# Genesis-Embodied-AI/ThinShellLab

Hardware: AMD Instinct MI355X
Metric: element-steps/s (fwd+adjoint), 100k-tri cloth; 1/2/4/8-GPU scaling (higher is better)
Workload: dtype f64

## Files before the change

### thinshelllab_amd/csrc/direct_host.hpp

```cpp
#pragma once
#include <array>
#include <chrono>

#include "k_direct.hpp"
#include "tsl_ctx.hpp"

#include <cerrno>
#include <fcntl.h>
#include <sys/file.h>
#include <sys/stat.h>
#include <unistd.h>
static void ds_flow_token_acquire(DirectSolver& d) {
  char bus[64] = "dev";
  if (hipDeviceGetPCIBusId(bus, sizeof(bus), d.device) != hipSuccess) { (void)hipGetLastError(); snprintf(bus, sizeof(bus), "dev%d", d.device); }
  for (char* q = bus; *q; q++) if (*q == ':' || *q == '/') *q = '_';
  d.flow_token = -1; d.flow_token_asked = d.n_factor;
  for (const char* dir : {"/dev/shm", "/tmp"}) {
    const std::string path = std::string(dir) + "/tsl_flow_" + bus;
    int fd = open(path.c_str(), O_RDWR | O_CLOEXEC);
    if (fd < 0 && errno == ENOENT) {
      fd = open(path.c_str(), O_CREAT | O_RDWR | O_CLOEXEC, 0666);
      if (fd < 0 && (errno == ENOENT || errno == ENOTDIR)) continue;
      if (fd < 0 && errno == EEXIST) fd = open(path.c_str(), O_RDWR | O_CLOEXEC);
    } else if (fd < 0 && errno == ENOTDIR) continue;
// ... 285 lines not shown
  if (d.cache_cap > 0) {
    const uint64_t key = ds_cons_key(cset);
    HIP_OK(hipStreamSynchronize(s));
    for (auto& sl : d.cache)
      if (sl->used && sl->key == key && sl->h_cset == cset) {
        ds_swap_slot(d, *sl);
        sl->used = d.plan_valid; sl->key = ds_cons_key(sl->h_cset); sl->stamp = ++d.cache_clock;
        d.plan_valid = true;
        d.n_plan_hits++; d.plan_gen++;
        if (c->group) TSL_TRY(group_ensure_arenas(c));
        if (c->verbose >= 2) fprintf(stderr, "[tsl] direct plan: cached plan reused (nc %d, %d supernodes)\n", c->nc, d.plan.sym.n_sn);
        return same_set_new_order();
      }
    if (d.plan_valid) {
      DsPlanSlot* dst = nullptr;
      for (auto& sl : d.cache) if (!sl->used) { dst = sl.get(); break; }
      if (!dst && (int)d.cache.size() < d.cache_cap) {
        d.cache.emplace_back(new DsPlanSlot());
        dst = d.cache.back().get();
        dst->plan.sym.copy_partition(d.plan.sym); dst->plan.threads = d.plan.threads; dst->plan.n_cu = d.plan.n_cu; dst->plan.split_small = d.plan.split_small; dst->plan.split_rem = d.plan.split_rem;
      }
      if (!dst) { for (auto& sl : d.cache) if (!dst || sl->stamp < dst->stamp) dst = sl.get(); }
      ds_swap_slot(d, *dst);
      dst->used = true; dst->key = ds_cons_key(dst->h_cset); dst->stamp = ++d.cache_clock;
      d.plan_valid = false;
      ds_cache_trim(d);
    }
  }
  const auto t0 = std::chrono::steady_clock::now();
  const int rc = d.plan.build(c->h_rows, d.row_ptr, cons.data(), c->nc);
  const auto t_build = std::chrono::steady_clock::now();
  if (rc) return tsl_fail("direct solver: inconsistent elimination tree (code %d)", rc);
  DirectPlan& P = d.plan;
  std::vector<int> vtxp(P.vtx.size());
  for (size_t i = 0; i < vtxp.size(); i++) vtxp[i] = c->h_rowpos[P.vtx[i]];
  HIP_OK(hipStreamSynchronize(s));
  const size_t nbk = P.blk_q.size();
  ds_pin_reset(d, 16 * nbk + 2 * sizeof(DsFrontDesc) * P.fr.size() + sizeof(DsChildRec) * P.ch_rec.size() +
                      4 * (P.level_sn.size() + P.pmap.size() + vtxp.size() + P.wl_front.size() + P.wl_row.size()) + 20 * (P.cgr_ent.size() + P.cgr_ptr.size()) + 64 * 256);
  TSL_TRY(ds_upload_grow(d.fr, P.fr, s, &d)); TSL_TRY(ds_upload_grow(d.level_sn, P.level_sn, s, &d)); TSL_TRY(ds_upload_grow(d.pmap, P.pmap, s, &d)); TSL_TRY(ds_upload_grow(d.ch_rec, P.ch_rec, s, &d));
  TSL_TRY(ds_upload_grow(d.vtx, vtxp, s, &d));
  {
    std::vector<int> src_v, ld_v;
    std::vector<long long> dst_v;
    int* src_l = (int*)ds_pin_take(d, 4 * nbk); int* ld_l = (int*)ds_pin_take(d, 4 * nbk); long long* dst_l = (long long*)ds_pin_take(d, 8 * nbk);
    if (!src_l || !ld_l || !dst_l) { src_v.resize(nbk); ld_v.resize(nbk); dst_v.resize(nbk); src_l = src_v.data(); ld_l = ld_v.data(); dst_l = dst_v.data(); }
    ds_parallel_for((int)((nbk + 4095) / 4096), P.n_threads(), 1, [&](int, int ch) {
      for (size_t i = (size_t)ch * 4096; i < std::min(nbk, (size_t)(ch + 1) * 4096); i++) { const int q = P.blk_q[i]; src_l[i] = d.h_c2s[q]; dst_l[i] = P.blk_dst[q]; ld_l[i] = P.blk_ld[q]; }
    });
    if (d.blk_dst.n < nbk) { if (d.blk_dst.alloc(nbk + nbk / 4 + 16)) return -1; }
    if (d.blk_ld.n < nbk) { if (d.blk_ld.alloc(nbk + nbk / 4 + 16)) return -1; }
    if (d.blk_q.n < nbk) { if (d.blk_q.alloc(nbk + nbk / 4 + 16)) return -1; }
    if (nbk > 0) {
      HIP_OK(hipMemcpyAsync(d.blk_dst.p, dst_l, 8 * nbk, hipMemcpyHostToDevice, s));
      HIP_OK(hipMemcpyAsync(d.blk_ld.p, ld_l, 4 * nbk, hipMemcpyHostToDevice, s));
      HIP_OK(hipMemcpyAsync(d.blk_q.p, src_l, 4 * nbk, hipMemcpyHostToDevice, s));
      if (!src_v.empty()) HIP_OK(hipStreamSynchronize(s));
    }
  }
  TSL_TRY(ds_upload_con(d, s));
  std::vector<DsFrontDesc> frl(P.level_sn.size());
  for (size_t i = 0; i < frl.size(); i++) frl[i] = P.fr[P.level_sn[i]];
  TSL_TRY(ds_upload_grow(d.frl, frl, s, &d));
  TSL_TRY(ds_upload_grow(d.wl_front, P.wl_front, s, &d)); TSL_TRY(ds_upload_grow(d.wl_row, P.wl_row, s, &d));
  if (c->group) TSL_TRY(group_ensure_arenas(c));
  else {
    if (d.prezero_pending && d.arena.n < (size_t)P.arena) { HIP_OK(hipEventSynchronize(d.ev_zero)); d.prezero_pending = false; }
    if (d.arena.n < (size_t)P.arena) { if (d.arena.alloc((size_t)P.arena + (size_t)P.arena / 8)) return tsl_fail("direct solver: out of device memory (%.2f GB of front panels)", P.arena * 8e-9); }
    if (d.sarena.n < (size_t)P.sarena) { if (d.sarena.alloc((size_t)P.sarena + (size_t)P.sarena / 8 + 16)) return tsl_fail("direct solver: out of device memory (%.2f GB of Schur complements)", P.sarena * 8e-9); }
    if (d.garena.n < (size_t)P.garena) { if (d.garena.alloc((size_t)P.garena + (size_t)P.garena / 8 + 16)) return tsl_fail("direct solver: out of device memory (G arena)"); }
    if (d.w.n < (size_t)P.ylen) { if (d.w.alloc((size_t)P.ylen + (size_t)P.ylen / 4 + 16)) return -1; }
  }
  if (d.scr.n < (size_t)P.scratch) { if (d.scr.alloc((size_t)P.scratch + (size_t)P.scratch / 8)) return -1; }
  HIP_OK(hipStreamSynchronize(s));
  d.h_cons.swap(cons); d.h_cset.swap(cset);
  d.plan_valid = true;
  d.numeric_valid = false;
  d.have_factor = false;
  d.n_plans++; d.plan_gen++;
  d.t_plan += std::chrono::duration<double>(std::chrono::steady_clock::now() - t0).count();
  if (c->verbose >= 2)
    fprintf(stderr, "[tsl] direct plan: %d supernodes, %d levels, %zu batches, %.2f + %.2f GB of panels + Schur complements, %.1f GFLOP per factorisation, nc %d; host %.2f ms (tree + maps %.2f)\n", P.sym.n_sn, P.n_levels, P.batches.size(), P.arena * 8e-9, P.sarena * 8e-9,
            P.flops * 1e-9, c->nc, 1e3 * std::chrono::duration<double>(std::chrono::steady_clock::now() - t0).count(), 1e3 * std::chrono::duration<double>(t_build - t0).count());
  if (c->verbose >= 2) fprintf(stderr, "[tsl]   plan phases (ms): tree %.2f, descriptors + parent maps %.2f, levels %.2f, static block map %.2f, contact map %.2f\n", P.phase_ms[0], P.phase_ms[1], P.phase_ms[2], P.phase_ms[3], P.phase_ms[4]);
  if (c->verbose >= 3)
    for (const DsBatch& b : P.batches) {
      fprintf(stderr, "[tsl]   level %2d: %5d fronts, pivots <= %4d, boundary <= %4d%s; fronts by padded pivot count:", b.level, b.count, b.max_pp, b.max_bp, ds_use_small(d, b) ? " (LDS kernel)" : "");
      for (int q = 0, run = 0; q < b.count; q++) {
        run++;
        if (q + 1 == b.count || P.fr[P.level_sn[b.first + q + 1]].pp != P.fr[P.level_sn[b.first + q]].pp) { fprintf(stderr, " %d x %d", run, P.fr[P.level_sn[b.first + q]].pp); run = 0; }
      }
      fprintf(stderr, "\n");
    }
  return 0;
}

static int direct_prezero(tsl_ctx* c) {
  DirectSolver& d = c->ds;
  if (!d.prezero || !d.plan_valid || d.arena.n == 0 || d.prezero_pending) return 0;
  if (d.zstream == nullptr) {
    HIP_OK(hipStreamCreateWithFlags(&d.zstream, hipStreamNonBlocking));
    HIP_OK(hipEventCreateWithFlags(&d.ev_zfork, hipEventDisableTiming));
    HIP_OK(hipEventCreateWithFlags(&d.ev_zero, hipEventDisableTiming));
  }
  HIP_OK(hipEventRecord(d.ev_zfork, c->stream));
  HIP_OK(hipStreamWaitEvent(d.zstream, d.ev_zfork, 0));
  d.prezero_n = (size_t)d.plan.arena_leaf;
  if (d.plan.leaf_ranges.empty()) HIP_OK(hipMemsetAsync(d.arena.p, 0, d.prezero_n * sizeof(double), d.zstream));
  else for (const auto& r : d.plan.leaf_ranges) HIP_OK(hipMemsetAsync(d.arena.p + r.first, 0, (size_t)r.second * sizeof(double), d.zstream));
  HIP_OK(hipEventRecord(d.ev_zero, d.zstream));
  d.prezero_pending = true;
  d.numeric_valid = false; d.have_factor = false;
  return 0;
}

static void ds_launch_gemv(hipStream_t s, const DsDev& D, DirectSolver& d, int o, int n, int mode, const double* vin, double* vout, int wide_from = -1) {
  if (n <= 0) return;
  if (wide_from >= 0) {
    const int n0 = wide_from - o, n1 = o + n - wide_from;
    if (n0 > 0) hipLaunchKernelGGL(k_ds_gemv, dim3(n0), dim3(256), 0, s, D, d.wl_front.p, d.wl_row.p, o, mode, vin, vout);
    if (n1 > 0) hipLaunchKernelGGL(k_ds_gemv_wide, dim3(4 * n1), dim3(256), 0, s, D, d.wl_front.p, d.wl_row.p, wide_from, mode, vin, vout);
    return;
  }
  if (d.gemv_wide_below > 0 && n < d.gemv_wide_below) hipLaunchKernelGGL(k_ds_gemv_wide, dim3(4 * n), dim3(256), 0, s, D, d.wl_front.p, d.wl_row.p, o, mode, vin, vout);
  else hipLaunchKernelGGL(k_ds_gemv, dim3(n), dim3(256), 0, s, D, d.wl_front.p, d.wl_row.p, o, mode, vin, vout);
}
static void ds_sweep_up_level(hipStream_t s, const DsDev& D, DirectSolver& d, int l, const double* r, double* z) {
  const DirectPlan& P = d.plan;
  const int o0 = P.wl_own_ptr[l], b0 = P.wl_bnd_ptr[l], o1 = P.wl_own_ptr[l + 1];
  ds_launch_gemv(s, D, d, o0, b0 - o0, 0, r, z, P.wl_own_wide.empty() ? -1 : P.wl_own_wide[l]);
  ds_launch_gemv(s, D, d, b0, o1 - b0, 1, (const double*)z, nullptr, P.wl_bnd_wide.empty() ? -1 : P.wl_bnd_wide[l]);
}
static int direct_factor(tsl_ctx* c, int stop_sn = -1, const char* dump_path = nullptr, const double* eager_r = nullptr, double* eager_z = nullptr) {
  DirectSolver& d = c->ds;
  hipStream_t s = c->stream;
  TSL_TRY(direct_plan(c));
  if (d.numeric_valid) return 0;
  d.eager_n = 0;
  const DirectPlan& P = d.plan;
  const DsDev D = ds_dev(c);
  if (d.prezero_pending) {
    HIP_OK(hipStreamWaitEvent(s, d.ev_zero, 0));
    d.prezero_pending = false;
    if (P.leaf_ranges.empty() && d.prezero_n < (size_t)P.arena_leaf) HIP_OK(hipMemsetAsync(d.arena.p + d.prezero_n, 0, ((size_t)P.arena_leaf - d.prezero_n) * sizeof(double), s));
  } else if (P.leaf_ranges.empty()) HIP_OK(hipMemsetAsync(d.arena.p, 0, (size_t)P.arena_leaf * sizeof(double), s));
  else for (const auto& r : P.leaf_ranges) HIP_OK(hipMemsetAsync(d.arena.p + r.first, 0, (size_t)r.second * sizeof(double), s));
  HIP_OK(hipMemsetAsync(d.bad.p, 0, 8 * sizeof(int), s));
  bool swept_at_root = false;
  int flow_wgs_sent = 0;
  auto invert_batch = [&](const DsBatch& b, hipStream_t bs, bool& flow_free) {
    const int lv0 = b.first, nf = b.count;
    const int tp = b.max_pp / DS_T;
    bool flowed = false;
    {
      const std::vector<DsBatch> pieces = ds_flow_pieces(d, P, b, flow_free, bs);
      std::vector<DsFlowArgs> fas(pieces.size());
      bool ready = !pieces.empty();
      for (size_t i = 0; ready && i < pieces.size(); i++) ready = ds_flow_prepare(d, P, pieces[i], true, fas[i], bs);
      if (ready) {
        for (size_t i = 0; i < pieces.size(); i++) { ds_flow_launch(bs, D, pieces[i].first, fas[i], d); d.n_flow++; flow_wgs_sent += fas[i].tile0[fas[i].nf]; }
        flowed = true; flow_free = false;
      }
    }
    if (flowed) {}
    else if (ds_use_small(d, b)) hipLaunchKernelGGL(k_ds_inv_small, dim3(nf), dim3(256), ds_small_lds(b.max_pp), bs, D, lv0, b.max_pp + 1);
    else {
      hipLaunchKernelGGL(k_ds_pivot0, dim3(nf), dim3(256), 0, bs, D, lv0);
      for (int k = 0; k < tp; k++) { const int na = P.act_n[b.act_off + k]; hipLaunchKernelGGL(k_ds_gj_step, dim3(na + na * tp * tp), dim3(256), 0, bs, D, lv0, k, tp, na); }
      hipLaunchKernelGGL(k_ds_gj_finish, dim3(tp, nf), dim3(256), 0, bs, D, lv0);
    }
  };
  auto run_batch = [&](const DsBatch& b, hipStream_t bs, bool& flow_free) {
    invert_batch(b, bs, flow_free);
    if (b.max_bp > 0) {
      ds_launch_gemm(bs, D, b, 0, d.xcd_map, d.g32_below);
      ds_launch_gemm(bs, D, b, 1, d.xcd_map);
    }
  };
  auto side_streams = [&]() -> int {
    if (d.fstream[0] == nullptr)
      for (int k = 0; k < DS_NSIDE; k++) { HIP_OK(hipStreamCreateWithFlags(&d.fstream[k], hipStreamNonBlocking)); HIP_OK(hipEventCreateWithFlags(&d.ev_fjoin[k], hipEventDisableTiming)); }
    if (d.ev_ffork == nullptr) HIP_OK(hipEventCreateWithFlags(&d.ev_ffork, hipEventDisableTiming));
    for (int k = 0; k < 5; k++) if (d.ev_la[k] == nullptr) HIP_OK(hipEventCreateWithFlags(&d.ev_la[k], hipEventDisableTiming));
    if (d.lastream == nullptr) {
      int lo = 0, hi = 0;
      HIP_OK(hipDeviceGetStreamPriorityRange(&lo, &hi));
      HIP_OK(hipStreamCreateWithPriority(&d.lastream, hipStreamNonBlocking, lo));
    }
    return 0;
  };
  const bool la_on = (d.lookahead & 1) && stop_sn < 0 && !P.blk_lmid.empty() && P.la_from < P.n_levels && ds_flow_token_held(d);
  if (la_on) TSL_TRY(side_streams());
  hipStream_t ls = d.lastream;
  enum { LA_W = 0, LA_GA = 1, LA_A = 2, LA_REST = 3, LA_DRAIN = 4 };
  for (size_t bi = 0; bi < P.batches.size();) {
    size_t be = bi;
    while (be < P.batches.size() && P.batches[be].level == P.batches[bi].level) be++;
    bool stop_here = false;
    if (stop_sn >= 0) for (int q = P.batches[bi].first; q < P.batches[be - 1].first + P.batches[be - 1].count; q++) stop_here |= P.level_sn[q] == stop_sn;
    const int lvl = P.batches[bi].level;
    const bool la_level = la_on && lvl >= P.la_from;
    const bool la_in = la_level && lvl > P.la_from;
    if (la_in) {
      ds_launch_level_start(c, s, D, lvl, 1, &P.batches[bi]);
      HIP_OK(hipStreamWaitEvent(ls, d.ev_la[LA_A], 0));
      ds_launch_level_start(c, ls, D, lvl, 2, &P.batches[bi]);
      HIP_OK(hipEventRecord(d.ev_la[LA_REST], ls));
    } else
    ds_launch_level_start(c, s, D, lvl);
    if (la_level) {
      const DsBatch& b = P.batches[bi];
      bool flow_free = true;
      if (la_in && ds_flow_wgs(P, b) > P.n_cu) {
        HIP_OK(hipEventRecord(d.ev_la[LA_DRAIN], ls));
        HIP_OK(hipStreamWaitEvent(s, d.ev_la[LA_DRAIN], 0));
      }
      invert_batch(b, s, flow_free);
      if (la_in && eager_r != nullptr && (d.lookahead & 2) && lvl >= P.n_levels - 3) {
        const int top = P.n_levels - 1;
        const int c0 = std::min((d.lookahead >> 2) & 7, top - 2);
        const int c1r = (d.lookahead >> 5) & 15, c1 = c1r == 0 ? top - 1 : std::min(std::max(c1r, c0), top - 1);
// ... 249 lines not shown
```

### thinshelllab_amd/csrc/direct_sym.hpp

```cpp
#pragma once
#include <algorithm>
#include <cstdint>
#include <cstdio>
#include <vector>

struct DsGrid { int v_offset, N, M; };
struct DsBlock { int v_offset, n_verts; };

struct DirectSym {
  int NV = 0;
  std::vector<int> c_order;
  std::vector<int> c_ptr;
  std::vector<int> c_lo;
  std::vector<int> c_grid;
  std::vector<int> c_pos;
  std::vector<int> c_sn;
  std::vector<DsBlock> blocks;
  std::vector<int> body_of;
  std::vector<std::vector<std::vector<int>>> b_sn;
  std::vector<int> loose;
  std::vector<int> order, epos, sn_of, sn_ptr;
  int n_sn = 0;
  int merge_sep = 16;
  bool merge_k = true;
  std::vector<std::vector<int>> bnd;
  std::vector<int> parent, level;
  int n_levels = 0;

  void copy_partition(const DirectSym& o) {
    NV = o.NV; c_order = o.c_order; c_ptr = o.c_ptr; c_lo = o.c_lo; c_grid = o.c_grid; c_pos = o.c_pos; c_sn = o.c_sn;
    blocks = o.blocks; body_of = o.body_of; b_sn = o.b_sn; loose = o.loose; merge_sep = o.merge_sep; merge_k = o.merge_k;
  }

  int own(int s) const { return sn_ptr[s + 1] - sn_ptr[s]; }

  int local(int s, int v) const {
    if (sn_of[v] == s) return epos[v] - sn_ptr[s];
    const auto& b = bnd[s];
    const int e = epos[v];
    int lo = 0, hi = (int)b.size();
    while (lo < hi) { const int m = (lo + hi) >> 1; if (epos[b[m]] < e) lo = m + 1; else hi = m; }
    if (lo < (int)b.size() && b[lo] == v) return own(s) + lo;
    return -1;
  }

  void build_partition(int nv, const std::vector<std::vector<int>>& adj, const std::vector<DsGrid>& grids, const std::vector<DsBlock>& blocks_in, int leaf_verts) {
    NV = nv;
    blocks = blocks_in;
    c_order.clear(); c_ptr.assign(1, 0); c_lo.clear(); c_grid.clear();
    c_pos.assign(nv, -1); c_sn.assign(nv, -1); body_of.assign(nv, -1); loose.clear();
    for (size_t b = 0; b < blocks.size(); b++)
      for (int v = blocks[b].v_offset; v < blocks[b].v_offset + blocks[b].n_verts; v++) body_of[v] = (int)b;
    b_sn.assign(blocks.size(), {});
    {
      std::vector<int> lab(nv, -1);
      for (size_t b = 0; b < blocks.size(); b++) {
        std::vector<int> region(blocks[b].n_verts);
        for (int k = 0; k < blocks[b].n_verts; k++) region[k] = blocks[b].v_offset + k;
        dissect_graph(adj, region, std::max(leaf_verts, 40), lab, b_sn[b]);
      }
    }
    std::vector<int> side(nv, 0);
    for (size_t gi = 0; gi < grids.size(); gi++) {
      const DsGrid& g = grids[gi];
      std::vector<int> region((size_t)(g.N + 1) * (g.M + 1));
      for (size_t k = 0; k < region.size(); k++) region[k] = g.v_offset + (int)k;
      dissect(g, (int)gi, adj, region, leaf_verts, side);
    }
    for (size_t q = 0; q < c_order.size(); q++) c_pos[c_order[q]] = (int)q;
    for (size_t s = 0; s + 1 < c_ptr.size(); s++)
      for (int q = c_ptr[s]; q < c_ptr[s + 1]; q++) c_sn[c_order[q]] = (int)s;
    for (int v = 0; v < nv; v++) if (c_pos[v] < 0 && body_of[v] < 0) loose.push_back(v);
  }

  void dissect_graph(const std::vector<std::vector<int>>& adj, std::vector<int>& region, int leaf, std::vector<int>& lab, std::vector<std::vector<int>>& out) {
    if (region.empty()) return;
    if ((int)region.size() <= leaf) { std::sort(region.begin(), region.end()); out.push_back(region); return; }
    std::vector<int> q;
    auto bfs = [&](int start) {
      for (int v : region) lab[v] = 0;
      q.clear(); q.push_back(start); lab[start] = 1;
      for (size_t h = 0; h < q.size(); h++)
        for (int u : adj[q[h]]) if (lab[u] == 0) { lab[u] = lab[q[h]] + 1; q.push_back(u); }
    };
    bfs(region[0]);
    if (q.size() < region.size()) {
      std::vector<int> comp(q), rest;
      for (int v : region) if (lab[v] == 0) rest.push_back(v);
      for (int v : region) lab[v] = -1;
      dissect_graph(adj, comp, leaf, lab, out);
      dissect_graph(adj, rest, leaf, lab, out);
      return;
    }
    bfs(q.back());
    const int nl = lab[q.back()];
    if (nl < 3) { for (int v : region) lab[v] = -1; std::sort(region.begin(), region.end()); out.push_back(region); return; }
    std::vector<int> cnt(nl + 2, 0);
    for (int v : region) cnt[lab[v]]++;
    int m = 2, acc = cnt[1];
    while (m < nl - 1 && 2 * (acc + cnt[m]) < (int)region.size()) { acc += cnt[m]; m++; }
    std::vector<int> A, B, S;
    for (int v : region) { if (lab[v] < m) A.push_back(v); else if (lab[v] > m) B.push_back(v); else S.push_back(v); }
    for (int v : region) lab[v] = -1;
    std::vector<int>().swap(region);
    dissect_graph(adj, A, leaf, lab, out);
    dissect_graph(adj, B, leaf, lab, out);
    std::sort(S.begin(), S.end());
    out.push_back(S);
  }

  void close_static(int lo, int grid) {
    if ((int)c_order.size() > c_ptr.back()) { c_ptr.push_back((int)c_order.size()); c_lo.push_back(lo); c_grid.push_back(grid); }
  }

  void dissect(const DsGrid& g, int gi, const std::vector<std::vector<int>>& adj, std::vector<int>& region, int leaf_verts, std::vector<int>& side, std::vector<int>* up = nullptr) {
    if (region.empty()) return;
    const int lo = (int)c_order.size();
    const int W = g.M + 1;
    int i0 = 1 << 30, i1 = -1, j0 = 1 << 30, j1 = -1;
    for (int v : region) { const int i = (v - g.v_offset) / W, j = (v - g.v_offset) % W; i0 = std::min(i0, i); i1 = std::max(i1, i); j0 = std::min(j0, j); j1 = std::max(j1, j); }
    const int ni = i1 - i0 + 1, nj = j1 - j0 + 1;
    if ((int)region.size() <= leaf_verts || (ni <= 3 && nj <= 3)) {
      std::sort(region.begin(), region.end());
      for (int v : region) c_order.push_back(v);
      close_static(lo, gi);
      return;
    }
    const bool along_i = ni >= nj;
    const int m = along_i ? (i0 + i1) / 2 : (j0 + j1) / 2;
    auto coord = [&](int v) { const int k = v - g.v_offset; return along_i ? k / W : k % W; };
    auto other = [&](int v) { const int k = v - g.v_offset; return along_i ? k % W : k / W; };
    std::vector<int> L, R, S;
    for (int v : region) { const int cv = coord(v); side[v] = cv < m ? 1 : cv > m + 1 ? 2 : 3; }
    std::vector<int> sep;
    for (int v : region) if (side[v] == 3) sep.push_back(v);
    std::stable_sort(sep.begin(), sep.end(), [&](int a, int b) { return coord(a) > coord(b); });
    for (int v : sep) {
      bool hasL = false, hasR = false;
      for (int u : adj[v]) { if (side[u] == 1) hasL = true; else if (side[u] == 2) hasR = true; }
      if (!hasL) side[v] = 2; else if (!hasR) side[v] = 1;
    }
    for (int v : region) { if (side[v] == 1) L.push_back(v); else if (side[v] == 2) R.push_back(v); else S.push_back(v); }
    for (int v : region) side[v] = 0;
    std::vector<int>().swap(region);
    std::vector<int> handed;
    dissect(g, gi, adj, L, leaf_verts, side, &handed);
    dissect(g, gi, adj, R, leaf_verts, side, &handed);
    std::sort(S.begin(), S.end(), [&](int a, int b) { return other(a) != other(b) ? other(a) < other(b) : coord(a) < coord(b); });
    if (up != nullptr && handed.empty() && (int)S.size() <= merge_sep) { up->insert(up->end(), S.begin(), S.end()); return; }
    for (int v : handed) c_order.push_back(v);
    for (int v : S) c_order.push_back(v);
    close_static(lo, gi);
  }

  void build_tree(const std::vector<std::vector<int>>& adj, const int* extra, int n_extra, int clique) {
    std::vector<std::vector<int>> xadj;
    std::vector<int> xidx(NV, -1);
    for (int e = 0; e < n_extra; e++)
      for (int a = 0; a < clique; a++) {
        const int va = extra[e * clique + a];
        if (xidx[va] < 0) { xidx[va] = (int)xadj.size(); xadj.emplace_back(); }
        for (int b = 0; b < clique; b++) if (b != a) xadj[xidx[va]].push_back(extra[e * clique + b]);
      }
    const int n_static = (int)c_ptr.size() - 1, END = n_static;
    const int nb = (int)blocks.size();
    std::vector<int> ins(nb, -1);
    std::vector<std::vector<int>> K(nb);
    for (int b = 0; b < nb; b++) {
      int pmin = 1 << 30, pmax = -1, grid = -1;
      bool to_end = false;
      for (int v = blocks[b].v_offset; v < blocks[b].v_offset + blocks[b].n_verts; v++) {
        if (xidx[v] < 0) continue;
        K[b].push_back(v);
        for (int u : xadj[xidx[v]]) {
          if (body_of[u] == b) continue;
          if (c_pos[u] < 0) { to_end = true; continue; }
          const int gu = c_grid[c_sn[u]];
          if (grid >= 0 && gu != grid) to_end = true;
          grid = gu;
          pmin = std::min(pmin, c_pos[u]); pmax = std::max(pmax, c_pos[u]);
        }
      }
      if (K[b].empty()) continue;
      if (to_end || pmax < 0) { ins[b] = END; continue; }
      int s = c_sn[c_order[pmax]];
      while (s < n_static && !(c_lo[s] <= pmin && c_ptr[s + 1] > pmax && c_grid[s] == grid)) s++;
      ins[b] = s;
    }
    order.clear(); sn_ptr.assign(1, 0);
    auto close_sn = [&]() { if ((int)order.size() > sn_ptr.back()) sn_ptr.push_back((int)order.size()); };
    for (int b = 0; b < nb; b++)
      for (const auto& sn : b_sn[b]) { for (int v : sn) if (xidx[v] < 0) order.push_back(v); close_sn(); }
    for (int v : loose) { order.push_back(v); close_sn(); }
    std::vector<std::vector<int>> at(n_static + 1);
    for (int b = 0; b < nb; b++) if (ins[b] >= 0) at[ins[b]].push_back(b);
    for (int s = 0; s <= n_static; s++) {
      for (int b : at[s]) for (int v : K[b]) order.push_back(v);
      if (!merge_k || s == n_static) close_sn();
      if (s < n_static) { for (int q = c_ptr[s]; q < c_ptr[s + 1]; q++) order.push_back(c_order[q]); close_sn(); }
    }
    n_sn = (int)sn_ptr.size() - 1;
    epos.assign(NV, 0); sn_of.assign(NV, 0);
    for (int p = 0; p < NV; p++) epos[order[p]] = p;
    for (int s = 0; s < n_sn; s++)
      for (int p = sn_ptr[s]; p < sn_ptr[s + 1]; p++) sn_of[order[p]] = s;
    bnd.assign(n_sn, {});
    parent.assign(n_sn, -1);
    level.assign(n_sn, 0);
    std::vector<std::vector<int>> children(n_sn);
    std::vector<int> mark(NV, -1);
    for (int s = 0; s < n_sn; s++) {
      std::vector<int>& b = bnd[s];
      auto visit = [&](int u) { if (sn_of[u] > s && mark[u] != s) { mark[u] = s; b.push_back(u); } };
      for (int p = sn_ptr[s]; p < sn_ptr[s + 1]; p++) {
        const int v = order[p];
        for (int u : adj[v]) visit(u);
        if (xidx[v] >= 0) for (int u : xadj[xidx[v]]) visit(u);
      }
      for (int c : children[s]) for (int u : bnd[c]) visit(u);
      std::sort(b.begin(), b.end(), [&](int x, int y) { return epos[x] < epos[y]; });
      if (!b.empty()) { parent[s] = sn_of[b[0]]; children[parent[s]].push_back(s); }
    }
    n_levels = 0;
    for (int s = 0; s < n_sn; s++) {
      int lv = 0;
      for (int c : children[s]) lv = std::max(lv, level[c] + 1);
      level[s] = lv;
      n_levels = std::max(n_levels, lv + 1);
    }
  }

  void stats(double* flops, double* front_doubles, int* max_front, int* max_p) const {
    double fl = 0, mem = 0;
    int mf = 0, mp = 0;
    for (int s = 0; s < n_sn; s++) {
      const double p = 3.0 * own(s), b = 3.0 * bnd[s].size();
      fl += 2.0 * p * p * p + 2.0 * p * p * b + 2.0 * p * b * b;
      mem += (p + b) * (p + b);
      mf = std::max(mf, (int)(p + b)); mp = std::max(mp, (int)p);
    }
    *flops = fl; *front_doubles = mem; *max_front = mf; *max_p = mp;
  }
};
```

### thinshelllab_amd/csrc/tsl_hip.hip

```cpp
#include <stdarg.h>
#include <cctype>
#include <chrono>
#include <mutex>

#include <array>
#include <map>

#include "k_cloth.hpp"
#include "k_contact.hpp"
#include "k_fem.hpp"
#include "k_mg.hpp"
#include "k_param.hpp"
#include "k_solver.hpp"
#include "tsl_ctx.hpp"

thread_local std::string g_tsl_err;
int tsl_fail(const char* fmt, ...) {
  char buf[1024];
  va_list ap;
  va_start(ap, fmt);
  vsnprintf(buf, sizeof(buf), fmt, ap);
  va_end(ap);
  g_tsl_err = buf;
  return -1;
// ... 1229 lines not shown
  if (c->nc > 0) std::swap(c->c_H.p, c->c_H_pc.p);
  const int rc = assemble(c, c->st_pos, c->st_prev, c->st_vel, c->st_ref, 2, nullptr);
  c->mg_omega_valid = false; c->mg_cinv_valid = false;
  c->bd_valid = false;
  int rc2 = 0;
  if (!rc) {
    if (body_active(c) && !c->bd_valid) rc2 = body_build_inverse(c);
    if (!rc2) rc2 = mg_setup_operators(c);
  }
  std::swap(c->vals.p, c->vals_pc.p);
  if (c->nc > 0) std::swap(c->c_H.p, c->c_H_pc.p);
  (void)s;
  if (rc || rc2) return -1;
  c->pc_separate = true;
  return 0;
}

static int ds_flow_lost(tsl_ctx* c, bool suspect, int note[8]) {
  const DirectSolver& d = c->ds;
  const bool forced = d.dbg == 21 || d.dbg == 22;
  if (!(suspect || forced) || !d.flow || d.n_flow <= 0) return 0;
  int ab = 0;
  HIP_OK(hipStreamSynchronize(c->stream));
  HIP_OK(hipMemcpy(&ab, d.bad.p + DS_FLOW_ABORT, sizeof(int), hipMemcpyDeviceToHost));
  if (!ab && !forced) return 0;
  for (int k = 0; k < 8; k++) note[k] = 0;
  (void)hipMemcpy(note, d.bad.p + DS_BAD_NOTE, 8 * sizeof(int), hipMemcpyDeviceToHost);
  return 1;
}

static int solve_perm(tsl_ctx* c, tsl_solve_stats* st, const tsl_solve_stats* first) {
  hipStream_t s = c->stream;
  const int NV = c->NV;
  const size_t n3 = 3 * (size_t)NV;
  const int gb = nblk(NV, 256);
  st->iters = 0; st->restarts = 0; st->flag = 0; st->rel_residual = 0; st->method = 0; st->attained = 0; st->backward_error = 0;
  c->last_xmax_valid = false;
  if (direct_enabled(c) && !c->ds_suspended) {
    DirectSolver& d = c->ds;
    if (!first && d.enable < 0 && !d.hard && c->n_tet == 0 && c->nc == 0) {
      c->ds_suspended = true; c->ds_probe = true;
      const int maxit_keep = c->cg_maxit;
      c->cg_maxit = std::min(c->cg_maxit, d.probe_cap);
      tsl_solve_stats s2;
      const int rc = solve_perm(c, &s2);
      c->cg_maxit = maxit_keep;
      c->ds_suspended = false; c->ds_probe = false;
      if (rc) return rc;
      if (s2.flag == 0) { *st = s2; return 0; }
      d.hard = true; d.hard_steps = 0;
      st->iters = s2.iters;
    }
    tsl_solve_stats sd = first ? *first : *st;
    auto direct_try = [&]() -> int {
      if (!d.numeric_valid) {
        TSL_TRY(direct_plan(c));
        TSL_TRY(direct_factor(c, -1, nullptr, c->v_b.p, c->v_x.p));
      }
      int rc_g = direct_refine(c, &sd, first != nullptr);
      if (rc_g == 0 && sd.flag != 1) { const int it0 = sd.iters; sd = *st; c->last_xmax_valid = false; rc_g = gmres(c, &sd, true); sd.iters += it0; }
      if (rc_g) return -1;
      int note[8];
      const int lost = ds_flow_lost(c, sd.flag != 1, note);
      if (lost < 0) return -1;
      if (lost) {
        const bool blame_la = (d.lookahead & 1) != 0 && d.n_flow_abort == 0 && d.dbg != 21;
        fprintf(stderr, "[tsl] k_ds_gj_flow: a workgroup waited in vain for a flag (launch not resident as a whole?): %s disabled for this context, refactorising "
                "(workgroup %d of %d gave up; %d of the %d workgroups of the factorisation's dataflow launches had started; flag value %d, epoch %d)\n",
                blame_la ? "\"direct_lookahead\"" : "\"direct_flow\"", note[2], note[1], note[0], d.flow_wgs_last, note[3], note[4]);
        const int flow_keep = d.flow;
        d.flow = 0; d.n_flow_abort++;
        if (blame_la) d.lookahead = 0;
        d.numeric_valid = false; d.have_factor = false;
        if (d.prezero_pending) { HIP_OK(hipStreamWaitEvent(c->stream, d.ev_zero, 0)); d.prezero_pending = false; }
        TSL_TRY(direct_factor(c));
        if (blame_la) d.flow = flow_keep;
        sd = *st; c->last_xmax_valid = false;
        TSL_TRY(direct_refine(c, &sd));
        if (sd.flag != 1) { const int it0 = sd.iters; sd = *st; c->last_xmax_valid = false; TSL_TRY(gmres(c, &sd, true)); sd.iters += it0; }
      }
      return 0;
    };
    if (direct_try() != 0) {
      if (d.enable == 1) return -1;
      (void)hipGetLastError();
      d.numeric_valid = false; d.have_factor = false; d.plan_valid = false;
      fprintf(stderr, "[tsl] direct solver set-up failed (%s): this solve runs on the iterative hierarchy%s\n", tsl_last_error(),
              ++d.n_setup_fail >= 3 ? "; direct path disabled for this context" : "");
      if (d.n_setup_fail >= 3) d.enable = 0;
      c->ds_suspended = true;
      const int rc = solve_perm(c, st);
      c->ds_suspended = false;
      if (rc == 0 && st->flag == 0) st->flag = 1;
      return rc;
    }
    if (sd.flag == 1) { *st = sd; st->flag = 0; st->method = 4; return 0; }
    if (c->verbose) {
      int nb[4] = {0, 0, 0, 0};
      (void)hipMemcpy(nb, d.bad.p, sizeof(nb), hipMemcpyDeviceToHost);
      fprintf(stderr, "[tsl] direct factorisation + GMRES did not converge (rel_residual %.2e, backward error %.2e after %d iterations, perturbed pivots %d / %d / %d in fronts of <= 128 / <= 512 / more pivots, nc %d): iterative fallback\n",
              sd.rel_residual, sd.backward_error, sd.iters, nb[1], nb[2], nb[3], c->nc);
      if (c->verbose > 1) {
        std::vector<int> lg(DS_BAD_NOTE);
        (void)hipMemcpy(lg.data(), d.bad.p, lg.size() * sizeof(int), hipMemcpyDeviceToHost);
        const int nl = std::min(lg[4], DS_BADLOG);
        static int n_dump = 0;
        if (const char* dir = getenv("TSL_DUMP_DIR")) if (nl > 0 && n_dump < 3) {
          char path[512];
          snprintf(path, sizeof(path), "%s/front_%d.bin", dir, n_dump++);
          d.numeric_valid = false;
          TSL_TRY(direct_factor(c, lg[8] >> 6, path));
        }
        for (int i = 0; i < nl; i++) {
          const int* L = &lg[8 + 4 * i];
          const int sn = L[0] >> 6, kt = L[0] & 63;
          const DsFrontDesc& f = d.plan.fr[sn];
          float am; memcpy(&am, L + 3, 4);
          const unsigned mask = (unsigned)L[1];
          const int first = __builtin_ctz(mask | 0x80000000u), row = kt * DS_T + first;
          const int vtx = row < f.p ? d.plan.vtx[f.vtx_off + row / 3] : -1;
          fprintf(stderr, "[tsl]   perturbed pivots: front %d (level %d, p %d, b %d, own verts %d) tile %d rows mask %08x, first row %d (vertex %d dof %d%s), tile max %.3e\n",
                  sn, d.plan.sym.level[sn], f.p, f.b, f.nv_own, kt, mask, row, vtx, row % 3, vtx >= 0 && d.plan.sym.body_of[vtx] >= 0 ? ", body" : "", am);
        }
      }
    }
    if (sd.rel_residual <= 1e-3) { *st = sd; st->flag = 3; st->method = 4; return 0; }
    c->ds_suspended = true;
    tsl_solve_stats s2;
    const int maxit_keep = c->cg_maxit;
    c->cg_maxit = std::min(c->cg_maxit, d.fallback_cap);
    HIP_OK(hipMemcpyAsync(c->v_t4.p, c->v_x.p, 3 * (size_t)c->NV * sizeof(double), hipMemcpyDeviceToDevice, c->stream));
    const int rc = solve_perm(c, &s2);
    c->cg_maxit = maxit_keep;
    c->ds_suspended = false;
    const bool sd_ok = std::isfinite(sd.rel_residual), s2_ok = rc == 0 && std::isfinite(s2.rel_residual);
    if (rc == 0 && s2.flag == 3 && !sd_ok && !s2_ok) return tsl_fail("linear solve: factorisation and iterative fallback both ended with a non-finite residual");
    if (rc == 0 && s2.flag == 3 && sd_ok && (!s2_ok || !(s2.rel_residual < sd.rel_residual))) {
      HIP_OK(hipMemcpyAsync(c->v_x.p, c->v_t4.p, 3 * (size_t)c->NV * sizeof(double), hipMemcpyDeviceToDevice, c->stream));
      *st = sd; st->iters = sd.iters + s2.iters; st->flag = 3; st->method = 4;
      return 0;
    }
    st->iters = sd.iters + s2.iters; st->restarts = s2.restarts + 1; st->rel_residual = s2.rel_residual; st->method = s2.method; st->attained = s2.attained;
    st->flag = s2.flag == 0 ? 1 : s2.flag;
    return rc;
  }
  TSL_TRY(block_jacobi_ensure(c));
  const bool warm = false;
  if (!warm) HIP_OK(hipMemsetAsync(c->v_x.p, 0, n3 * sizeof(double), s));
  HIP_OK(hipMemsetAsync(c->scal.p, 0, sizeof(SolverScalars), s));
  hipLaunchKernelGGL(k_dot, dim3(DOT_BLOCKS), dim3(256), 0, s, n3, c->v_b.p, c->v_b.p, &SC(c)->bb, DOT_SCRATCH(c));
  TSL_TRY(read_scal(c));
  const double bb = HSC(c)->bb;
  if (!(bb > 0)) return 0;
  const double tol2 = c->cg_tol * c->cg_tol * bb;
  bool need_fallback = false, indefinite = false;
  int total_it = 0;
  const int ncb = c->nc > 0 ? nblk(c->nc, 64) : 0;
  if (body_active(c) && !c->bd_valid) TSL_TRY(body_build_inverse(c));
  const bool bd = body_active(c) && c->bd_valid;
  const int n_rz = gb + (bd ? c->bd_wg : 0);
  double rr_prev_outer = 1e300;
  for (int outer = 0; outer < 20; outer++) {
    PcgScal hs;
    memset(&hs, 0, sizeof(hs));
    hs.bb = bb; hs.thresh2 = 0.25 * tol2; hs.n_part1 = c->n_slices; hs.n_part2 = n_rz;
    HIP_OK(hipMemcpyAsync(c->scal.p, &hs, sizeof(PcgScal), hipMemcpyHostToDevice, s));
// ... 1498 lines not shown
```

Baseline: 525,600.

## Reuse constraint-free elimination tree boundaries when rebuilding the direct solver plan

Caches the elimination tree and supernode boundary sets computed without contact constraints, and on each replan only recomputes boundaries for static supernodes touched by contact cliques and their ancestors. Clean supernodes copy their cached boundary lists, which is meant to cut host-side symbolic planning time per step. Scratch workspaces are kept across calls to avoid reallocations. It also adds a state check for when the cached tree applies, and resets eager_n earlier. The cost is added complexity and a correctness risk if the dirty propagation misses a case.

Result: no change. 522,000 (-0.7%).

```diff
diff --git a/thinshelllab_amd/csrc/direct_host.hpp b/thinshelllab_amd/csrc/direct_host.hpp
--- a/thinshelllab_amd/csrc/direct_host.hpp
+++ b/thinshelllab_amd/csrc/direct_host.hpp
@@ -391,7 +391,8 @@
   if (c->verbose >= 2)
     fprintf(stderr, "[tsl] direct plan: %d supernodes, %d levels, %zu batches, %.2f + %.2f GB of panels + Schur complements, %.1f GFLOP per factorisation, nc %d; host %.2f ms (tree + maps %.2f)\n", P.sym.n_sn, P.n_levels, P.batches.size(), P.arena * 8e-9, P.sarena * 8e-9,
             P.flops * 1e-9, c->nc, 1e3 * std::chrono::duration<double>(std::chrono::steady_clock::now() - t0).count(), 1e3 * std::chrono::duration<double>(t_build - t0).count());
-  if (c->verbose >= 2) fprintf(stderr, "[tsl]   plan phases (ms): tree %.2f, descriptors + parent maps %.2f, levels %.2f, static block map %.2f, contact map %.2f\n", P.phase_ms[0], P.phase_ms[1], P.phase_ms[2], P.phase_ms[3], P.phase_ms[4]);
+  if (c->verbose >= 1) fprintf(stderr, "[tsl]   plan phases (ms): tree %.2f (%d of %d boundaries kept from the constraint-free tree), descriptors + parent maps %.2f, levels %.2f, static block map %.2f, contact map %.2f, uploads %.2f\n",
+                               P.phase_ms[0], P.sym.n_reused, P.sym.n_sn, P.phase_ms[1], P.phase_ms[2], P.phase_ms[3], P.phase_ms[4], 1e3 * std::chrono::duration<double>(std::chrono::steady_clock::now() - t_build).count());
   if (c->verbose >= 3)
     for (const DsBatch& b : P.batches) {
       fprintf(stderr, "[tsl]   level %2d: %5d fronts, pivots <= %4d, boundary <= %4d%s; fronts by padded pivot count:", b.level, b.count, b.max_pp, b.max_bp, ds_use_small(d, b) ? " (LDS kernel)" : "");
@@ -443,9 +444,9 @@
 static int direct_factor(tsl_ctx* c, int stop_sn = -1, const char* dump_path = nullptr, const double* eager_r = nullptr, double* eager_z = nullptr) {
   DirectSolver& d = c->ds;
   hipStream_t s = c->stream;
+  d.eager_n = 0;
   TSL_TRY(direct_plan(c));
   if (d.numeric_valid) return 0;
-  d.eager_n = 0;
   const DirectPlan& P = d.plan;
   const DsDev D = ds_dev(c);
   if (d.prezero_pending) {
diff --git a/thinshelllab_amd/csrc/direct_sym.hpp b/thinshelllab_amd/csrc/direct_sym.hpp
--- a/thinshelllab_amd/csrc/direct_sym.hpp
+++ b/thinshelllab_amd/csrc/direct_sym.hpp
@@ -26,10 +26,18 @@
   std::vector<std::vector<int>> bnd;
   std::vector<int> parent, level;
   int n_levels = 0;
+  bool reuse = true;
+  int st_state = 0;
+  std::vector<int> st_parent;
+  std::vector<int> st_bptr, st_bnd;
+  int n_reused = 0;
+  std::vector<std::vector<int>> w_xadj, w_K, w_at, w_children;
+  std::vector<int> w_xidx, w_touched, w_ins, w_mark, w_dirty, w_dyn;
 
   void copy_partition(const DirectSym& o) {
     NV = o.NV; c_order = o.c_order; c_ptr = o.c_ptr; c_lo = o.c_lo; c_grid = o.c_grid; c_pos = o.c_pos; c_sn = o.c_sn;
     blocks = o.blocks; body_of = o.body_of; b_sn = o.b_sn; loose = o.loose; merge_sep = o.merge_sep; merge_k = o.merge_k;
+    reuse = o.reuse; st_state = o.st_state; st_parent = o.st_parent; st_bptr = o.st_bptr; st_bnd = o.st_bnd;
   }
 
   int own(int s) const { return sn_ptr[s + 1] - sn_ptr[s]; }
@@ -47,6 +55,7 @@
   void build_partition(int nv, const std::vector<std::vector<int>>& adj, const std::vector<DsGrid>& grids, const std::vector<DsBlock>& blocks_in, int leaf_verts) {
     NV = nv;
     blocks = blocks_in;
+    st_state = 0; st_parent.clear(); st_bptr.clear(); st_bnd.clear();
     c_order.clear(); c_ptr.assign(1, 0); c_lo.clear(); c_grid.clear();
     c_pos.assign(nv, -1); c_sn.assign(nv, -1); body_of.assign(nv, -1); loose.clear();
     for (size_t b = 0; b < blocks.size(); b++)
@@ -153,7 +162,7 @@
     close_static(lo, gi);
   }
 
-  void build_tree(const std::vector<std::vector<int>>& adj, const int* extra, int n_extra, int clique) {
+  void build_tree_scratch(const std::vector<std::vector<int>>& adj, const int* extra, int n_extra, int clique) {
     std::vector<std::vector<int>> xadj;
     std::vector<int> xidx(NV, -1);
     for (int e = 0; e < n_extra; e++)
@@ -230,6 +239,134 @@
     }
   }
 
+  void build_static_tree(const std::vector<std::vector<int>>& adj) {
+    const int n_static = (int)c_ptr.size() - 1;
+    st_state = -1;
+    if (!loose.empty() || n_static == 0) return;
+    for (int v = 0; v < NV; v++)
+      for (int u : adj[v]) if ((c_pos[v] >= 0) != (c_pos[u] >= 0) || body_of[v] != body_of[u]) return;
+    build_tree_scratch(adj, nullptr, 0, 4);
+    const int base = n_sn - n_static;
+    if (base < 0) return;
+    for (int s = 0; s < n_static; s++) if (sn_ptr[base + s + 1] - sn_ptr[base + s] != c_ptr[s + 1] - c_ptr[s] || order[sn_ptr[base + s]] != c_order[c_ptr[s]]) return;
+    st_parent.assign(n_static, -1); st_bptr.assign(n_static + 1, 0); st_bnd.clear();
+    for (int s = 0; s < n_static; s++) {
+      if (parent[base + s] >= 0) { if (parent[base + s] < base) return; st_parent[s] = parent[base + s] - base; }
+      for (int u : bnd[base + s]) { if (c_pos[u] < 0) return; st_bnd.push_back(u); }
+      st_bptr[s + 1] = (int)st_bnd.size();
+    }
+    st_state = 1;
+  }
+
+  void build_tree(const std::vector<std::vector<int>>& adj, const int* extra, int n_extra, int clique) {
+    n_reused = 0;
+    if (!reuse) { build_tree_scratch(adj, extra, n_extra, clique); return; }
+    if (st_state == 0) build_static_tree(adj);
+    if (st_state < 0) { build_tree_scratch(adj, extra, n_extra, clique); return; }
+    std::vector<std::vector<int>>& xadj = w_xadj;
+    std::vector<int>& xidx = w_xidx;
+    if ((int)xidx.size() != NV) { xidx.assign(NV, -1); w_touched.clear(); }
+    for (int v : w_touched) xidx[v] = -1;
+    w_touched.clear();
+    int nx = 0;
+    for (int e = 0; e < n_extra; e++)
+      for (int a = 0; a < clique; a++) {
+        const int va = extra[e * clique + a];
+        if (xidx[va] < 0) { xidx[va] = nx++; w_touched.push_back(va); if ((int)xadj.size() < nx) xadj.emplace_back(); xadj[nx - 1].clear(); }
+        for (int b = 0; b < clique; b++) if (b != a) xadj[xidx[va]].push_back(extra[e * clique + b]);
+      }
+    const int n_static = (int)c_ptr.size() - 1, END = n_static;
+    const int nb = (int)blocks.size();
+    std::vector<int>& ins = w_ins;
+    ins.assign(nb, -1);
+    std::vector<std::vector<int>>& K = w_K;
+    K.resize(nb);
+    for (int b = 0; b < nb; b++) {
+      K[b].clear();
+      int pmin = 1 << 30, pmax = -1, grid = -1;
+      bool to_end = false;
+      for (int v = blocks[b].v_offset; v < blocks[b].v_offset + blocks[b].n_verts; v++) {
+        if (xidx[v] < 0) continue;
+        K[b].push_back(v);
+        for (int u : xadj[xidx[v]]) {
+          if (body_of[u] == b) continue;
+          if (c_pos[u] < 0) { to_end = true; continue; }
+          const int gu = c_grid[c_sn[u]];
+          if (grid >= 0 && gu != grid) to_end = true;
+          grid = gu;
+          pmin = std::min(pmin, c_pos[u]); pmax = std::max(pmax, c_pos[u]);
+        }
+      }
+      if (K[b].empty()) continue;
+      if (to_end || pmax < 0) { ins[b] = END; continue; }
+      int s = c_sn[c_order[pmax]];
+      while (s < n_static && !(c_lo[s] <= pmin && c_ptr[s + 1] > pmax && c_grid[s] == grid)) s++;
+      ins[b] = s;
+    }
+    order.clear(); sn_ptr.assign(1, 0);
+    auto close_sn = [&]() { if ((int)order.size() > sn_ptr.back()) sn_ptr.push_back((int)order.size()); };
+    for (int b = 0; b < nb; b++)
+      for (const auto& sn : b_sn[b]) { for (int v : sn) if (xidx[v] < 0) order.push_back(v); close_sn(); }
+    for (int v : loose) { order.push_back(v); close_sn(); }
+    std::vector<std::vector<int>>& at = w_at;
+    at.resize(n_static + 1);
+    for (auto& a : at) a.clear();
+    for (int b = 0; b < nb; b++) if (ins[b] >= 0) at[ins[b]].push_back(b);
+    std::vector<int>& dyn = w_dyn;
+    dyn.clear();
+    for (int s = 0; s <= n_static; s++) {
+      for (int b : at[s]) for (int v : K[b]) order.push_back(v);
+      if (!merge_k || s == n_static) close_sn();
+      if (s < n_static) { for (int q = c_ptr[s]; q < c_ptr[s + 1]; q++) order.push_back(c_order[q]); close_sn(); dyn.resize(sn_ptr.size() - 1, -1); dyn.back() = s; }
+    }
+    n_sn = (int)sn_ptr.size() - 1;
+    dyn.resize(n_sn, -1);
+    epos.resize(NV); sn_of.resize(NV);
+    for (int p = 0; p < NV; p++) epos[order[p]] = p;
+    for (int s = 0; s < n_sn; s++)
+      for (int p = sn_ptr[s]; p < sn_ptr[s + 1]; p++) sn_of[order[p]] = s;
+    std::vector<int>& dirty = w_dirty;
+    dirty.assign(n_static, 0);
+    for (int v : w_touched) if (c_sn[v] >= 0) dirty[c_sn[v]] = 1;
+    for (int b = 0; b < nb; b++) if (ins[b] >= 0 && ins[b] < n_static) dirty[ins[b]] = 1;
+    for (int s = 0; s < n_static; s++) if (dirty[s] && st_parent[s] >= 0) dirty[st_parent[s]] = 1;
+    if ((int)bnd.size() > n_sn) bnd.resize(n_sn);
+    bnd.resize(n_sn);
+    parent.assign(n_sn, -1);
+    level.assign(n_sn, 0);
+    std::vector<std::vector<int>>& children = w_children;
+    if ((int)children.size() < n_sn) children.resize(n_sn);
+    for (int s = 0; s < n_sn; s++) children[s].clear();
+    std::vector<int>& mark = w_mark;
+    mark.assign(NV, -1);
+    for (int s = 0; s < n_sn; s++) {
+      std::vector<int>& b = bnd[s];
+      b.clear();
+      const int ss = dyn[s];
+      if (ss >= 0 && !dirty[ss]) {
+        b.assign(st_bnd.begin() + st_bptr[ss], st_bnd.begin() + st_bptr[ss + 1]);
+        n_reused++;
+      } else {
+        auto visit = [&](int u) { if (sn_of[u] > s && mark[u] != s) { mark[u] = s; b.push_back(u); } };
+        for (int p = sn_ptr[s]; p < sn_ptr[s + 1]; p++) {
+          const int v = order[p];
+          for (int u : adj[v]) visit(u);
+          if (xidx[v] >= 0) for (int u : xadj[xidx[v]]) visit(u);
+        }
+        for (int c : children[s]) for (int u : bnd[c]) visit(u);
+        std::sort(b.begin(), b.end(), [&](int x, int y) { return epos[x] < epos[y]; });
+      }
+      if (!b.empty()) { parent[s] = sn_of[b[0]]; children[parent[s]].push_back(s); }
+    }
+    n_levels = 0;
+    for (int s = 0; s < n_sn; s++) {
+      int lv = 0;
+      for (int c : children[s]) lv = std::max(lv, level[c] + 1);
+      level[s] = lv;
+      n_levels = std::max(n_levels, lv + 1);
+    }
+  }
+
   void stats(double* flops, double* front_doubles, int* max_front, int* max_p) const {
     double fl = 0, mem = 0;
     int mf = 0, mp = 0;
diff --git a/thinshelllab_amd/csrc/tsl_hip.hip b/thinshelllab_amd/csrc/tsl_hip.hip
--- a/thinshelllab_amd/csrc/tsl_hip.hip
+++ b/thinshelllab_amd/csrc/tsl_hip.hip
@@ -1335,6 +1335,7 @@
       return 0;
     };
     if (direct_try() != 0) {
+      d.eager_n = 0;
       if (d.enable == 1) return -1;
       (void)hipGetLastError();
       d.numeric_valid = false; d.have_factor = false; d.plan_valid = false;
```
